# uguryagmur/RealTimeObjectDetection

Hardware: AMD Instinct MI355X
Metric: frames/sec YOLOv3 608x608 bs=8 (Darknet.forward + write_results; 2 batches in flight, write_results_async on a second stream) (higher is better)
Workload: dtype f16x2-split (3 MFMA products, f32 accumulate); 1 GPU; YOLOv3 cfg 608x608 batch=8 per GPU, split-f16 MFMA conv + fused head + GPU NMS (BASELINE configs[2]); precision=f16s3, tiles=autotune (this run), parallelism=frame-shard x1, in_flight_batches=2, detections_last_step=1699, candidates_last_step=1914, f16_range_overflow=False

## Files before the change

### realtimeobjectdetection_amd/csrc/conv_f16s3_common.h

```cpp
#pragma once
#include "rtod_internal.h"
#include <type_traits>

namespace rtod {

typedef float f32x4 __attribute__((ext_vector_type(4)));
typedef _Float16 f16x8 __attribute__((ext_vector_type(8)));
typedef unsigned int u32x4 __attribute__((ext_vector_type(4)));

constexpr int HBK = 32;
constexpr unsigned OOB = 0x80000000u;


template <int N> __device__ __forceinline__ void vmcnt() {
    static_assert(0 <= N && N <= 63, "vmcnt range");
    asm volatile("s_waitcnt vmcnt(%0)" :: "n"(N) : "memory");
}

template <int OFF = 0> __device__ __forceinline__ u32x4 buffer_load_b128(const __amdgpu_buffer_rsrc_t rsrc, unsigned voffset, unsigned soffset) {
    u32x4 v;
    asm volatile("buffer_load_dwordx4 %0, %1, %2, %3 offen offset:%4" : "=v"(v) : "v"(voffset), "s"(rsrc), "s"(soffset), "n"(OFF) : "memory");
    return v;
}

// ... 169 lines not shown
        if (kg == 1) return;
#pragma unroll
        for (int i = 0; i < TM; ++i)
#pragma unroll
            for (int j = 0; j < TN; ++j) {
                const f32x4 o = T[base + (i * TN + j) * 64];
#pragma unroll
                for (int e = 0; e < 4; ++e) acc[i][j][e] += o[e];
            }
    }
    float amax = 0.f;
    _Float16* const oh = reinterpret_cast<_Float16*>(a.out) + a.out_coff;
    const _Float16* const rh = reinterpret_cast<const _Float16*>(a.res) + a.res_coff;
#pragma unroll
    for (int P = 0; P < NP; ++P) {
        const int c0 = cbase + 32 * P + 8 * lh;
        const bool cok = c0 < a.Cout;
        const int cc = cok ? c0 : 0;
        f16x8 rq_h[RES ? TM : 1], rq_l[RES ? TM : 1];
        if constexpr (RES) {
#pragma unroll
            for (int i = 0; i < TM; ++i) {
                const int m = mrow[i];
                const bool ok = m >= 0 && cok;
                const _Float16* q = rh + (int64_t)(ok ? m : 0) * 2 * a.res_ldc + cc;
                rq_h[i] = ok ? *reinterpret_cast<const f16x8*>(q) : f16x8{0, 0, 0, 0, 0, 0, 0, 0};
                rq_l[i] = ok ? *reinterpret_cast<const f16x8*>(q + a.res_ldc) : f16x8{0, 0, 0, 0, 0, 0, 0, 0};
            }
        }
        f32x4 iv0 = *reinterpret_cast<const f32x4*>(a.inv_scale + cc), iv1 = *reinterpret_cast<const f32x4*>(a.inv_scale + cc + 4);
        f32x4 bs0 = *reinterpret_cast<const f32x4*>(a.bias + cc), bs1 = *reinterpret_cast<const f32x4*>(a.bias + cc + 4);
#pragma unroll
        for (int i = 0; i < TM; ++i) {
            const int m = mrow[i];
            f16x8 ph, pl;
#pragma unroll
            for (int e = 0; e < 8; ++e) {
                const float s = e < 4 ? acc[i][2 * P][e] : acc[i][2 * P + 1][e - 4];
                float v = s * ((e < 4 ? iv0[e] : iv1[e - 4]) * SPLIT_SCALE) + (e < 4 ? bs0[e] : bs1[e - 4]) * SPLIT_SCALE;
                if (a.leaky) v = v > 0.f ? v : v * 0.1f;
                if constexpr (RES) v += (float)rq_h[i][e] + (float)rq_l[i][e];
                _Float16 h, l;
                split_f16(v, h, l, amax);
                ph[e] = h; pl[e] = l;
            }
            if (m >= 0 && cok) {
                _Float16* q = oh + (int64_t)m * 2 * a.out_ldc + c0;
                store_act16(q, ph, false);
                store_act16(q + a.out_ldc, pl, false);
            }
        }
    }
    split_overflow_report(a.ovf, amax);
}

constexpr int epi_row_group(int bm, int wm, int rg_max) {
    int best = wm;
    for (int r = wm; r <= bm && r <= rg_max; r += wm) if (bm % r == 0) best = r;
    return best;
}


template <int BM, int BN, int WM, int WN, int NT, int EPI, int SMEM_BYTES, int KG = 1, bool PRE = false, bool F16 = false, bool RAW = false>
__device__ __forceinline__ void conv_f16s3_epilogue(const ConvArgs& a, f32x4 (&acc)[WM / 16][WN / 16], unsigned char* smem,
                                                    int bm, int bn, int tid, int wm, int wn, int lr, int lh, int M, int kg = 0,
                                                    const float* pre_bias = nullptr, const float* pre_inv = nullptr) {
    constexpr int MT = 16, TM = WM / MT, TN = WN / MT;
    constexpr bool PW = EPI == EPI_SPLIT_PW || EPI == EPI_SPLIT_RES_PW;
    constexpr bool RES = EPI == EPI_SPLIT_RES || EPI == EPI_SPLIT_RES_PW;
    static_assert(!(F16 && PW), "plain-f16 plans host no pointwise conv");
    static_assert(!RAW || (EPI == EPI_SPLIT && !F16), "raw-sum instances: no shortcut, decode, hosted pointwise conv or plain-f16 store");
    constexpr int TS = PW ? BN + 4 : BN;
    constexpr int T2S = PW_MAX_COUT + 4;
    constexpr int RG_MAX = SMEM_BYTES / ((TS + (PW ? T2S : 0)) * 4);
    constexpr int RG = epi_row_group(BM, WM, RG_MAX);
    static_assert(RG >= WM && BM % RG == 0, "epilogue row group");
    static_assert(RG * (TS + (PW ? T2S : 0)) * 4 <= SMEM_BYTES, "epilogue tile exceeds the kernel's LDS");
    float* T = reinterpret_cast<float*>(smem);
    const int hw = a.Ho * a.Wo;
#ifdef RTOD_DIAG
    const bool st_plain = (a.dbg & 8) != 0;
#else
    constexpr bool st_plain = false;
#endif
    float amax = 0.f;
    constexpr int PWK = PW_MAX_K / 32;
    f16x8 b2h[PW ? PWK : 1], b2l[PW ? PWK : 1];
    float bias2 = 0.f, inv2 = 0.f;
    int pw_n2t = 1, pw_j = 0;
    if constexpr (PW) {
        pw_n2t = a.pw_cout / 16;
        pw_j = (tid >> 6) % pw_n2t;
        const int n2 = pw_j * 16 + (tid & 15);
        const _Float16* w2h = a.pw_wh + (int64_t)n2 * 32 + ((tid & 63) >> 4) * 8;
        const _Float16* w2l = a.pw_wl + (int64_t)n2 * 32 + ((tid & 63) >> 4) * 8;
#pragma unroll
        for (int ks = 0; ks < PWK; ++ks) {
            const bool ok = ks * 32 < a.pw_k;
            b2h[ks] = ok ? *reinterpret_cast<const f16x8*>(w2h + (int64_t)ks * a.pw_npad * 32) : f16x8{0, 0, 0, 0, 0, 0, 0, 0};
            b2l[ks] = ok ? *reinterpret_cast<const f16x8*>(w2l + (int64_t)ks * a.pw_npad * 32) : f16x8{0, 0, 0, 0, 0, 0, 0, 0};
        }
        bias2 = a.pw_bias[n2] * SPLIT_SCALE; inv2 = a.pw_inv_scale[n2] * SPLIT_SCALE;
    }
    const float escale = (EPI == EPI_DECODE || RAW) ? 1.0f : SPLIT_SCALE;
    constexpr int GPR_ = BN / 8;
    constexpr int NG = (RG * GPR_ + NT - 1) / NT;
// ... 174 lines not shown
```

### realtimeobjectdetection_amd/csrc/conv_pwd_f16s3.hip

```cpp
#include "conv_bandd_common.h"

namespace rtod {

template <int BM, int NW, int NST, int MINW, int EPI>
__global__ __launch_bounds__(NW * 64, MINW)
void conv_pwd_f16s3_kernel(const ConvArgs a, const int grid_m, const int grid_n) {
    constexpr bool F16 = epi_f16(EPI);
    constexpr int LB = F16 ? 2 : 4, LP = F16 ? 1 : 2;
    constexpr int BN = NW * 32, NT = NW * 64, TM = BM / 16, TN = 2;
    constexpr int SLAB = BM * 256;
    constexpr int NP = BM / 8;
    constexpr int NPP = (NP + NW - 1) / NW;
    static_assert(BM % 16 == 0 && NPP >= 1 && NPP <= 8, "slab pieces per wave");
    static_assert(NST >= 2 && NST <= 4, "ring depth");
    constexpr int RG = BM * BN * 4 <= 32768 ? BM : (BM / 2) * BN * 4 <= 32768 ? BM / 2 : BM / 4;
    constexpr int WAIT_B = 2 * LB + LP * NPP;
    constexpr int WAIT_SLAB = 2 * LB + (NST - 2) * (LP * NPP + 2 * LB);
    constexpr int WAIT_SLAB_PRO = 2 * LB + (NST - 2) * LP * NPP;

    extern __shared__ __attribute__((aligned(16))) unsigned char smem[];
    const int nwg = grid_m * grid_n;
    int bid = blockIdx.x;
    if (!a.xcd_by_n) bid = xcd_remap(bid, nwg);
    const int bm = bid / grid_n, bn = bid - bm * grid_n;
    const int tid = (int)threadIdx.x;
    const int wave = __builtin_amdgcn_readfirstlane(tid >> 6), lane = tid & 63;
    const int lr = lane & 15, lh = lane >> 4;
    const int M = a.B * a.Hi * a.Wi;
    const int m0 = bm * BM;
    const unsigned PS = (unsigned)a.in_ldc * 4u;
    const unsigned lo_plane = (unsigned)a.in_ldc * 2u;

    const __amdgpu_buffer_rsrc_t rs_a = buffer_rsrc(a.in, a.in_bytes);
    const __amdgpu_buffer_rsrc_t rs_wh = buffer_rsrc(a.w_hi, a.w_bytes);
    const __amdgpu_buffer_rsrc_t rs_wl = buffer_rsrc(a.w_lo, a.w_bytes);
    const unsigned lds0 = (unsigned)(size_t)smem;
    const int NS = a.Cin / 64;

    unsigned dma_vo[NPP];
#pragma unroll
    for (int k = 0; k < NPP; ++k) {
        const int p = wave + k * NW;
        const int r = lane >> 3;
        const int m = m0 + p * 8 + r;
        dma_vo[k] = (p < NP && m < M) ? (unsigned)m * PS + (unsigned)(a.in_coff + (((lane & 7) ^ r) << 3)) * 2u : OOB;
    }
    auto dma_slab = [&](int js) __attribute__((always_inline)) {
        const bool live = js < NS;
        const unsigned soff = (unsigned)js * 128u;
        const unsigned base = lds0 + (unsigned)((js % NST) * SLAB);
#pragma unroll
        for (int k = 0; k < NPP; ++k) {
            const int p = wave + k * NW;
            const unsigned dst = p < NP ? base + (unsigned)((p >> 1) * 4096 + (p & 1) * 1024) : lds0 + (unsigned)(NST * SLAB);
            if constexpr (F16) lds_dma(rs_a, live ? dma_vo[k] : OOB, soff, dst);
// ... 34 lines not shown
        if constexpr (!F16) l = *reinterpret_cast<lds_f16x8*>((unsigned)(o + 4096 * i + 2048));
    };

#pragma unroll
    for (int s = 0; s < NST - 1; ++s) dma_slab(s);
    load_b(0, Bq[0]);
    load_b(1, Bq[1]);

    __builtin_amdgcn_s_setprio(2);
    auto slab_body = [&](int j, auto par_c) __attribute__((always_inline)) {
        constexpr int par = decltype(par_c)::value;
        asm volatile("" : "+v"(xq0), "+v"(xq1));
        if (j < NST - 1) vmcnt<WAIT_SLAB_PRO>(); else vmcnt<WAIT_SLAB>();
        __builtin_amdgcn_sched_barrier(0);
        __builtin_amdgcn_s_barrier();
        dma_slab(j + NST - 1);
        const int slotoff = (int)lds0 + (j % NST) * SLAB;
        read_unit(0, 0, slotoff, Ah[0], Al[0]);
        read_unit(1 / TM, 1 % TM, slotoff, Ah[1], Al[1]);
        __builtin_amdgcn_sched_barrier(0);
#pragma unroll
        for (int u = 0; u < 2 * TM; ++u) {
            const int q = u / TM, i = u % TM;
            if (i == 0) {
                if (q == 0) load_b(2 * j + 2, Bq[(2 * par + 2) % 4]); else load_b(2 * j + 3, Bq[(2 * par + 3) % 4]);
                vmcnt<WAIT_B>();
                if (q == 0) tie_bset<F16>(Bq[2 * par]); else tie_bset<F16>(Bq[2 * par + 1]);
                __builtin_amdgcn_sched_barrier(0);
            }
            if (u + 2 < 2 * TM) read_unit((u + 2) / TM, (u + 2) % TM, slotoff, Ah[(u + 2) % 3], Al[(u + 2) % 3]);
            const f16x8 ah = Ah[u % 3], al = Al[u % 3];
#pragma unroll
            for (int jn = 0; jn < TN; ++jn) {
                const f16x8 bh = __builtin_bit_cast(f16x8, Bq[2 * par + q][jn][0]);
                if constexpr (F16) { acc[i][jn] = __builtin_amdgcn_mfma_f32_16x16x32_f16(ah, bh, acc[i][jn], 0, 0, 0); continue; }
                const f16x8 bl = __builtin_bit_cast(f16x8, Bq[2 * par + q][jn][1]);
                acc[i][jn] = __builtin_amdgcn_mfma_f32_16x16x32_f16(al, bh, acc[i][jn], 0, 0, 0);
                acc[i][jn] = __builtin_amdgcn_mfma_f32_16x16x32_f16(ah, bl, acc[i][jn], 0, 0, 0);
                acc[i][jn] = __builtin_amdgcn_mfma_f32_16x16x32_f16(ah, bh, acc[i][jn], 0, 0, 0);
            }
            __builtin_amdgcn_sched_barrier(0);
        }
    };
#pragma unroll 1
    for (int j = 0; j < NS; j += 2) {
        slab_body(j, std::integral_constant<int, 0>{});
        if (j + 1 < NS) slab_body(j + 1, std::integral_constant<int, 1>{});
    }
    vmcnt<0>();
    tie_bset<F16>(Bq[0]); tie_bset<F16>(Bq[1]); tie_bset<F16>(Bq[2]); tie_bset<F16>(Bq[3]);
    __builtin_amdgcn_sched_barrier(0);
    __builtin_amdgcn_s_setprio(0);

    bandd_epilogue<BM, BN, BM, 32, NT, RG, epi_kind(EPI) == EPI_SPLIT_RES, 1, F16, epi_raw(EPI)>(a, acc, smem, bm, bn, tid, 0, wn, lr, lh, M, 0);
}

template <int BM, int NW, int NST, int MINW>
static int launch_pwd(const ConvArgs& a, hipStream_t s) {
    constexpr int BN = NW * 32, NT = NW * 64;
    constexpr int RG = BM * BN * 4 <= 32768 ? BM : (BM / 2) * BN * 4 <= 32768 ? BM / 2 : BM / 4;
    const int M = a.B * a.Ho * a.Wo;
    const int gm = (M + BM - 1) / BM, gn = (a.Cout + BN - 1) / BN;
    ConvArgs ax = a;
    ax.xcd_by_n = (gn % 8 == 0 && (int64_t)a.Cout * a.K > (int64_t)M * a.Cin) ? 1 : 0;
    constexpr int ring_bytes = NST * BM * 256 + ((BM / 8) % NW ? 4096 : 0), epi_bytes = RG * BN * 4;
    constexpr int lds = ring_bytes > epi_bytes ? ring_bytes : epi_bytes;
    static_assert(lds <= 160 * 1024, "LDS");
    const int fe = a.f16 ? 1 : 0;
    auto k_res = fe ? conv_pwd_f16s3_kernel<BM, NW, NST, MINW, EPI_SPLIT_RES | EPI_F16> : conv_pwd_f16s3_kernel<BM, NW, NST, MINW, EPI_SPLIT_RES>;
    auto k_plain = fe ? conv_pwd_f16s3_kernel<BM, NW, NST, MINW, EPI_SPLIT | EPI_F16> : conv_pwd_f16s3_kernel<BM, NW, NST, MINW, EPI_SPLIT>;
    auto k_raw = conv_pwd_f16s3_kernel<BM, NW, NST, MINW, EPI_SPLIT | EPI_RAW>;
    if constexpr (lds > 64 * 1024) {
        static std::atomic<unsigned long long> attr_done[3] = {{0}, {0}, {0}};
        if (a.raw_out) { if (int rc = lds_opt_in(attr_done[2], lds, "conv_pwd_f16s3", k_raw)) return rc; }
        else if (int rc = lds_opt_in(attr_done[fe], lds, "conv_pwd_f16s3", k_res, k_plain)) return rc;
    }
    if (a.raw_out) {
        hipLaunchKernelGGL(k_raw, dim3(gm * gn), dim3(NT), lds, s, ax, gm, gn);
        return hip_fail(hipGetLastError(), "conv_pwd_f16s3 launch");
    }
    if (a.res) hipLaunchKernelGGL(k_res, dim3(gm * gn), dim3(NT), lds, s, ax, gm, gn);
    else hipLaunchKernelGGL(k_plain, dim3(gm * gn), dim3(NT), lds, s, ax, gm, gn);
    return hip_fail(hipGetLastError(), "conv_pwd_f16s3 launch");
}

#define RTOD_PWD_TILES(X) \
    X(0, 64, 4, 3, 3) X(1, 32, 4, 3, 3) X(2, 128, 4, 3, 1) X(3, 64, 8, 3, 1) X(4, 64, 4, 2, 3) X(5, 32, 4, 4, 3) X(6, 96, 4, 2, 3) X(7, 96, 4, 3, 2) X(8, 48, 4, 3, 3) X(9, 48, 4, 4, 3) X(10, 64, 2, 2, 4)

#define RTOD_X_INFO(idx, bm, nw, nst, minw) {bm, nw * 32, "conv_pwd_f16s3<" #bm "x" #nw "w,r" #nst ">"},
static const ConvVariantInfo kPwdModes[PWD_MODES] = { RTOD_PWD_TILES(RTOD_X_INFO) };
#undef RTOD_X_INFO
const ConvVariantInfo& conv_pwd_mode_info(int idx) { return kPwdModes[idx < 0 || idx >= PWD_MODES ? 0 : idx]; }

bool conv_pwd_supported(int ksize, int stride, int pad, int cin) { return ksize == 1 && stride == 1 && pad == 0 && cin >= 64 && cin % 64 == 0; }

int conv_pwd_kernel_name(int idx, int epi, char* buf, size_t len) {
#define RTOD_X_NAME(i, bm, nw, nst, minw) \
    if (idx == i) return snprintf(buf, len, "void rtod::conv_pwd_f16s3_kernel<" #bm ", " #nw ", " #nst ", " #minw ", %d>(rtod::ConvArgs, int, int)", epi);
    RTOD_PWD_TILES(RTOD_X_NAME)
#undef RTOD_X_NAME
    return -1;
}

int launch_conv_pwd_f16s3(const ConvArgs& a, int idx, hipStream_t s) {
    if (int rc = check_split_conv_args(a, "launch_conv_pwd", true)) return rc;
    if (!conv_pwd_supported(a.kh, a.stride, a.pad, a.Cin) || a.kw != 1 || a.Ho != a.Hi || a.Wo != a.Wi || a.dec.enabled || a.pw_wh) {
        set_error("launch_conv_pwd: unsupported shape (k=%d s=%d pad=%d Cin=%d)", a.kh, a.stride, a.pad, a.Cin); return RTOD_E_ARG;
    }
    if (a.in_ldc % 8 || a.in_coff % 8 || a.K != a.Kpad || a.K != a.Cin || a.Npad % 128) { set_error("launch_conv_pwd: bad view / K"); return RTOD_E_ARG; }
    if (a.raw_out && (a.f16 || a.res)) { set_error("launch_conv_pwd: a raw-sum launch carries no shortcut and no plain-f16 store"); return RTOD_E_ARG; }
    if (a.raw_out && a.raw_ld != a.Npad) { set_error("launch_conv_pwd: raw-sum rows are Npad floats in this family (raw_ld %d, Npad %d)", a.raw_ld, a.Npad); return RTOD_E_ARG; }
    switch (idx) {
#define RTOD_X_CASE(i, bm, nw, nst, minw) case i: return launch_pwd<bm, nw, nst, minw>(a, s);
        RTOD_PWD_TILES(RTOD_X_CASE)
#undef RTOD_X_CASE
    }
    set_error("launch_conv_pwd: mode %d unsupported", idx);
    return RTOD_E_ARG;
}

}
```

### realtimeobjectdetection_amd/csrc/plan_tiles.cpp

```cpp
#include "plan.h"

#include <algorithm>
#include <mutex>

namespace rtod {

int Plan::choose_variant(const Layer& L, int batch) const {
    if (opt_force_f32_variant >= 0 && opt_force_f32_variant < CV_COUNT) return opt_force_f32_variant;
    if (L.cout <= 32) return CV_128x32;
    if (L.cout <= 64) return CV_128x64;
    const int64_t M = (int64_t)batch * L.hout * L.wout;
    const int64_t big = ((M + 127) / 128) * ((L.cout + 127) / 128);
    return big >= 512 ? CV_128x128 : CV_64x64;
}

int Plan::f32_slice_mode(const Launch& l, int batch, int variant) const {
    const PackedConv& pc = convs[l.conv_slot];
    if (pc.split || pc.stem || pc.slice_chunks <= 0) return 0;
    const Layer& L = layers[l.layer];
    const ConvVariantInfo& vi = conv_variant_info(variant);
    const int64_t M = (int64_t)batch * L.hout * L.wout;
    const int64_t tiles = ((M + vi.bm - 1) / vi.bm) * ((L.cout + vi.bn - 1) / vi.bn);
    const int64_t S = (pc.Kpad / 32 + pc.slice_chunks - 1) / pc.slice_chunks;
    return (opt_k_slice_workgroups && d_scratch && tiles < 512 && S * M * pc.Npad <= scratch_floats) ? 2 : 1;
}

bool Plan::tile_legal(const Launch& l, int v) const {
    const TileRef t = family_of(v);
    if (!t || l.kind != LK_CONV || l.conv_slot < 0 || !convs[l.conv_slot].split) return false;
    const PackedConv& pc = convs[l.conv_slot];
    const Layer& L = layers[l.layer];
    if (precision == 2 && !t.f16()) return false;
    if (raw_launch(l) && !t.raw()) return false;
    if (pc.narrow || t.is(TF_C16)) return pc.narrow && t.is(TF_C16);
    if (pc.ks_chunks > 0 || t.is(TF_KS)) return pc.ks_chunks > 0 && t.is(TF_KS);
    if (pc.band) return t.is(TF_BAND) && conv_band_mode_valid(t.mode, L.cin, L.hin, L.win);
    const bool hosts_pw = form(&l - &launches[0]).guest >= 0, plain = l.out_layer != -2 && !hosts_pw, same_map = L.hout == L.hin && L.wout == L.win;
    switch (t.fam->id) {
        case TF_GENERIC: return !(hosts_pw && t.fam->info(t.mode).bn < L.cout);
        case TF_BAND: return t.bandd_wide() && opt_band_kernel && plain && same_map && pc.Npad % 128 == 0 && pc.K == pc.Kpad &&
                             conv_bandd_wide_supported(L.size, L.stride, L.pad, pc.cin_p, L.win);
        case TF_RING: return !hosts_pw && L.act <= 1;
        case TF_PWD: return opt_pwd_kernel && plain && same_map && conv_pwd_supported(L.size, L.stride, L.pad, pc.cin_p);
        case TF_PATCH: return plain && L.act <= 1 && L.hout == L.hin && conv_patch_supported(L.size, L.stride, L.pad, L.cin, L.cout) &&
                              conv_patch_mode_valid(t.mode, L.cin, L.cout);
    }
    return false;
}

int Plan::default_tile(const Launch& l, int batch) const {
    const PackedConv& pc = convs[l.conv_slot];
    const Layer& L = layers[l.layer];
    const int64_t M = (int64_t)batch * L.hout * L.wout;
    if (pc.narrow) return tile_id(TF_C16, conv_c16_default_mode(L.cout, M));
    if (pc.ks_chunks > 0) return tile_id(TF_KS, ((M + 63) / 64) * ((L.cout + 63) / 64) < 512 ? 1 : 0);
    if (pc.band) {
        if (precision != 2 && !raw_launch(l)) return tile_id(TF_BAND, conv_band_default_mode(L.cin, L.hin, L.win));
        const TileFamily& B = tile_family(TF_BAND);
        for (int m = 0; m < B.modes; ++m) if (tile_legal(l, B.base + m)) return B.base + m;
        return B.base + B.f16_from;
    }
    const int64_t gn = (L.cout + 127) / 128;
    const int g = L.cout <= 64 ? HV_128x64 : ((M + 127) / 128) * gn >= 512 ? HV_128x128 : ((M + 63) / 64) * gn >= 512 ? HV_64x128 : HV_64x64;
    return tile_legal(l, g) ? g : HV_128x128_8W;
}

int Plan::variant_for(const Launch& l, int batch) const {
    int want = opt_force_f16s3_variant;
    if (want < 0) {
        auto it = tuned.find(batch);
        const size_t idx = &l - &launches[0];
        if (it != tuned.end() && idx < it->second.size()) want = it->second[idx];
    }
    int v = want >= 0 && tile_legal(l, want) ? want : default_tile(l, batch);
    if (family_of(v).ks_sched_b() && !(opt_k_slice_workgroups && ks_sched_b_fits(l, batch))) --v;
    return v;
}

std::vector<int> Plan::tile_candidates(const Launch& l, int batch) const {
    static const int kOrder[TF_COUNT] = {TF_GENERIC, TF_PATCH, TF_BAND, TF_PWD, TF_RING, TF_C16, TF_KS};
    const int cout = layers[l.layer].cout;
    const bool ks_b = opt_k_slice_workgroups && ks_sched_b_fits(l, batch);
    std::vector<int> cand;
    for (int f : kOrder) {
        if ((f == TF_RING && !opt_ring_kernel) || (f == TF_PATCH && !opt_patch_kernel)) continue;
        const TileFamily& F = tile_family(f);
        for (int m = 0; m < F.modes; ++m) {
            const int bn = F.info(m).bn;
            const bool too_wide = f == TF_GENERIC || f == TF_RING ? bn > 64 && bn > 2 * ((cout + 63) / 64 * 64)
                                : f == TF_PATCH ? bn > 64 && bn > cout
                                : f == TF_PWD ? bn > 128 && bn > (cout + 127) / 128 * 128 : false;
            if (too_wide || (family_of(F.base + m).ks_sched_b() && !ks_b) || !tile_legal(l, F.base + m)) continue;
            cand.push_back(F.base + m);
        }
    }
    return cand;
}

int Plan::launch_split_variant(ConvArgs& a, const PackedConv& pc, int v, hipStream_t s) const {
    const TileRef t = family_of(v);
    if (!t) { set_error("variant %d is no split-f16 tile", v); return RTOD_E_STATE; }
    if (precision == 2 && !t.f16()) { set_error("variant %d has no plain-f16 instance", v); return RTOD_E_STATE; }
    if (a.raw_out && !t.raw()) { set_error("variant %d has no raw-sum instance", v); return RTOD_E_STATE; }
    if (pc.narrow != t.is(TF_C16)) {
        set_error(pc.narrow ? "variant %d requested for a narrow (Cin = 16) layer" : "narrow variant %d requested for a layer without tap-major weights", v);
        return RTOD_E_STATE;
    }
    if ((pc.ks_chunks > 0) != t.is(TF_KS)) {
        set_error(pc.ks_chunks > 0 ? "variant %d requested for a K-sliced layer" : "K-sliced variant %d requested for a layer that is not sliced", v);
        return RTOD_E_STATE;
    }
    if (pc.band != t.is(TF_BAND) && !(t.bandd_wide() && !pc.band)) {
        set_error(pc.band ? "variant %d requested for a band layer" : "band variant %d requested for a layer without band weights", v);
        return RTOD_E_STATE;
    }
    if (t.is(TF_KS)) {
        a.slice_chunks = pc.ks_chunks;
        a.partial = nullptr; a.partial_floats = 0;
        if (t.ks_sched_b()) { a.partial = d_scratch; a.partial_floats = scratch_floats; }
    }
    return t.fam->launch(a, t.mode, s);
}

static std::mutex g_tune_mutex;
static std::map<std::vector<int>, int> g_tune_memo;

int Plan::tune_launch(size_t li, ConvArgs& a, int batch, hipStream_t s) {
    const Launch& l = launches[li];
    const Layer& L = layers[l.layer];
    const bool pw = a.pw_wh != nullptr;
    const std::vector<int> key = {L.cin, L.cout, L.size, L.stride, L.hout, L.wout, l.in2_layer >= 0, l.out_layer == -2, pw ? a.pw_cout : 0,
                                  convs[l.conv_slot].band ? 1 : 0, opt_ring_kernel ? 1 : 0, opt_patch_kernel ? 1 : 0, opt_pwd_kernel ? 1 : 0, L.act,
                                  precision, L.hin, L.win, L.pad, convs[l.conv_slot].ks_chunks, opt_k_slice_workgroups ? 1 : 0,
                                  a.raw_out ? 1 : 0};
    auto it = tune_cache.find(key);
    if (it != tune_cache.end()) { tuning[li] = it->second; return RTOD_OK; }
    std::vector<int> gkey = key; gkey.push_back(device); gkey.push_back(batch);
    {
        std::lock_guard<std::mutex> lock(g_tune_mutex);
        auto git = g_tune_memo.find(gkey);
        if (git != g_tune_memo.end()) { tuning[li] = git->second; tune_cache[key] = git->second; return RTOD_OK; }
    }
    hipEvent_t e0, e1;
    RTOD_HIP(hipEventCreate(&e0)); RTOD_HIP(hipEventCreate(&e1));
    const std::vector<int> cand = tile_candidates(l, batch);
    int best_v = variant_for(l, batch);
    int rc = RTOD_OK;
    auto time_variant = [&](int v, int reps, int per, float& out_ms) -> int {
        out_ms = 1e30f;
        for (int rep = 0; rep < reps; ++rep) {
            (void)hipEventRecord(e0, s);
            for (int r = 0; r < per; ++r) { const int q = launch_split_variant(a, convs[l.conv_slot], v, s); if (q) return q; }
            (void)hipEventRecord(e1, s);
            if (hipEventSynchronize(e1) != hipSuccess) return hip_fail(hipGetLastError(), "autotune sync");
            float ms = 0.f; (void)hipEventElapsedTime(&ms, e0, e1);
            out_ms = std::min(out_ms, ms / per);
        }
        return RTOD_OK;
    };
    std::vector<std::pair<float, int>> ranked;
    for (int v : cand) {
        rc = launch_split_variant(a, convs[l.conv_slot], v, s);
        if (rc) break;
        float ms; rc = time_variant(v, 3, 2, ms);
        if (rc) break;
        ranked.push_back({ms, v});
    }
    if (!rc && !ranked.empty()) {
        std::sort(ranked.begin(), ranked.end());
        const size_t top = std::min<size_t>(3, ranked.size());
        std::vector<float> fin(top, 1e30f);
        for (int round = 0; round < 5 && !rc; ++round)
            for (size_t t = 0; t < top && !rc; ++t) {
                float ms; rc = time_variant(ranked[t].second, 2, 4, ms);
                fin[t] = std::min(fin[t], ms);
            }
        if (!rc) best_v = ranked[std::min_element(fin.begin(), fin.end()) - fin.begin()].second;
    }
    (void)hipEventDestroy(e0); (void)hipEventDestroy(e1);
    if (rc) return rc;
    tuning[li] = best_v;
    tune_cache[key] = best_v;
    { std::lock_guard<std::mutex> lock(g_tune_mutex); g_tune_memo[gkey] = best_v; }
    return RTOD_OK;
}

int Plan::set_tiles(int batch, const int* variants, int count) {
// ... 27 lines not shown
```

### realtimeobjectdetection_amd/csrc/rtod_internal.h

```cpp
#pragma once
#include <hip/hip_runtime.h>
#if defined(RTOD_STAMPS) && !defined(RTOD_DIAG)
#define RTOD_DIAG 1
#endif
#include <algorithm>
#include <atomic>
#include <cstdint>
#include <cstdio>
#include <string>
#include <vector>

#include "../../include/rtod.h"

namespace rtod {

void set_error(const char* fmt, ...);
int hip_fail(hipError_t e, const char* what);

#define RTOD_HIP(expr)                                              \
    do {                                                            \
        hipError_t _e = (expr);                                     \
        if (_e != hipSuccess) return ::rtod::hip_fail(_e, #expr);   \
    } while (0)

// ... 98 lines not shown
}
__device__ __forceinline__ __amdgpu_buffer_rsrc_t buffer_rsrc(const void* p, unsigned bytes) {
    return __builtin_amdgcn_make_buffer_rsrc(const_cast<void*>(p), 0, bytes, 0x00020000);
}
__device__ __forceinline__ int xcd_remap(int id, int n) {
    const int q = n >> 3, r = n & 7, xcd = id & 7;
    return (xcd < r ? xcd * (q + 1) : r * (q + 1) + (xcd - r) * q) + (id >> 3);
}
#endif

constexpr int EPI_F16 = 8;
constexpr int EPI_RAW = 16;

enum ConvVariant { CV_128x128 = 0, CV_128x64 = 1, CV_64x64 = 2, CV_128x32 = 3, CV_COUNT };
struct ConvVariantInfo { int bm, bn; const char* name; };
const ConvVariantInfo& conv_variant_info(int v);
int conv_f32_kernel_name(int variant, char* buf, size_t len);
int launch_conv(const ConvArgs& a, int variant, hipStream_t s);
int conv_f32_slices(const ConvArgs& a);
enum ConvF16Variant { HV_128x128 = 0, HV_128x64 = 1, HV_64x64 = 2, HV_64x128 = 3, HV_256x128 = 4, HV_128x256 = 5, HV_128x128_8W = 6, HV_128x64_8W = 7, HV_256x128_16W = 8,
                      HV_192x128_8W = 9, HV_96x128_8W = 10, HV_192x128_12W = 11, HV_COUNT };
const ConvVariantInfo& conv_f16s3_variant_info(int v);
int conv_f16s3_kernel_name(int variant, int epi, char* buf, size_t len);
int launch_conv_f16s3(const ConvArgs& a, int variant, hipStream_t s);
bool conv_band_supported(int ksize, int stride, int pad, int cin, int w_in);
constexpr int BANDD_MODES = 9;
constexpr int BAND_LDS_MODES = 11;
constexpr int BAND_MODES = BAND_LDS_MODES + BANDD_MODES;
constexpr int BAND_K2_MODE0 = 7;
const ConvVariantInfo& conv_bandd_mode_info(int idx);
int conv_bandd_mode_kg(int idx);
constexpr int BANDD_WIDE_MODE = BAND_LDS_MODES + 7;
bool conv_bandd_wide_supported(int ksize, int stride, int pad, int cin, int w_in);
int conv_bandd_kernel_name(int idx, int epi, char* buf, size_t len);
int launch_conv_bandd_f16s3(const ConvArgs& a, int idx, hipStream_t s);
int conv_band_layer_kg(int cin, int h, int w);
bool conv_band_mode_valid(int mode, int cin, int h, int w);
int conv_band_default_mode(int cin, int h, int w);
const ConvVariantInfo& conv_band_mode_info(int mode);
int conv_band_kernel_name(int mode, int epi, char* buf, size_t len);
int launch_conv_band_f16s3(const ConvArgs& a, int mode, hipStream_t s);
constexpr int BAND_VARIANT_BASE = 50;
constexpr int RING_MODES = 8;
constexpr int RING_VARIANT_BASE = 70;
const ConvVariantInfo& conv_ring_mode_info(int mode);
int conv_ring_kernel_name(int mode, int epi, char* buf, size_t len);
int launch_conv_ring_f16s3(const ConvArgs& a, int mode, hipStream_t s);
constexpr int PWD_MODES = 11;
constexpr int PWD_VARIANT_BASE = 90;
bool conv_pwd_supported(int ksize, int stride, int pad, int cin);
const ConvVariantInfo& conv_pwd_mode_info(int mode);
int conv_pwd_kernel_name(int mode, int epi, char* buf, size_t len);
int launch_conv_pwd_f16s3(const ConvArgs& a, int mode, hipStream_t s);
constexpr int STEM2_VARIANT = 130;
bool conv_stem2_supported(int k0, int s0, int p0, int cin0, int cout0, int k1, int s1, int p1, int cout1, int pw_cout);
int conv_stem2_kernel_name(int pw, char* buf, size_t len);
int launch_conv_stem2_f16s3(const float* x, int B, int H, int W, const _Float16* w0h, const _Float16* w0l, const float* inv0, const float* bias0,
                            int leaky0, const ConvArgs& c1, hipStream_t s);
constexpr int PATCH_MODES = 5;
constexpr int PATCH_WRES_MODE = 4;
bool conv_patch_mode_valid(int mode, int cin, int cout);
constexpr int PATCH_VARIANT_BASE = 110;
bool conv_patch_supported(int ksize, int stride, int pad, int cin, int cout);
const ConvVariantInfo& conv_patch_mode_info(int mode);
int conv_patch_kernel_name(int mode, int epi, char* buf, size_t len);
int launch_conv_patch_f16s3(const ConvArgs& a, int mode, hipStream_t s);

constexpr int C16_MODES = 4;
constexpr int C16_VARIANT_BASE = 140;
constexpr bool conv_c16_supported(int cin) { return cin == 16; }
const ConvVariantInfo& conv_c16_mode_info(int mode);
int conv_c16_default_mode(int cout, int64_t m);
int conv_c16_kernel_name(int mode, int epi, char* buf, size_t len);
int launch_conv_c16_f16s3(const ConvArgs& a, int mode, hipStream_t s);

constexpr int KS_TILES = 3;
constexpr int KS_MODES = 2 * KS_TILES;
constexpr int KS_VARIANT_BASE = 150;
constexpr int64_t KS_SCRATCH_FLOATS = 8ll << 20;
const ConvVariantInfo& conv_ks_mode_info(int mode);
int conv_ks_slices(const ConvArgs& a);
int conv_ks_kernel_name(int mode, int epi, char* buf, size_t len);
int launch_conv_ks_f16s3(const ConvArgs& a, int mode, hipStream_t s);

enum TileFamilyId { TF_GENERIC = 0, TF_BAND, TF_RING, TF_PWD, TF_PATCH, TF_C16, TF_KS, TF_COUNT };
struct TileFamily {
    int id, base, modes;
    int f16_from;
    int raw_from;
    const ConvVariantInfo& (*info)(int mode);
    int (*kernel_name)(int mode, int epi, char* buf, size_t len);
    int (*launch)(const ConvArgs& a, int mode, hipStream_t s);
};
struct TileRef {
    const TileFamily* fam; int mode;
    explicit operator bool() const { return fam != nullptr; }
    bool is(int family) const { return fam && fam->id == family; }
    bool f16() const { return fam && mode >= fam->f16_from; }
    bool raw() const { return fam && mode >= fam->raw_from; }
    bool ks_sched_b() const { return is(TF_KS) && (mode & 1); }
    bool bandd_wide() const { return is(TF_BAND) && mode == BANDD_WIDE_MODE; }
};
TileRef family_of(int v);
const TileFamily& tile_family(int family);
inline int tile_id(int family, int mode) { return tile_family(family).base + mode; }

int launch_conv_stem(const float* x_nchw, const float* w, const float* bias, const View& out, int B, int H, int W,
                     int Ho, int Wo, int stride, int Cout, int leaky, hipStream_t s);
int launch_conv_stem_split(const float* x_nchw, const _Float16* wh, const _Float16* wl, const float* inv_scale, const float* bias,
                           const View& out, int B, int H, int W, int Ho, int Wo, int stride, int Cout, int leaky, int32_t* ovf, hipStream_t s);
bool conv_stem16_supported(int ksize, int stride, int pad, int cin, int cout, int act);
int launch_conv_stem16_f16s3(const float* x_nchw, const _Float16* wh, const _Float16* wl, const float* inv_scale, const float* bias,
                             const View& out, int B, int H, int W, int act, int pool, int32_t* ovf, hipStream_t s);
int launch_conv_stem16_raw(const float* x_nchw, const _Float16* wh, const _Float16* wl, const float* inv_scale, const View& raw, int B, int H, int W, hipStream_t s);
int launch_prep_image(const unsigned char* img, int h, int w, int bgr, int inp_dim, float* out, hipStream_t s);
int launch_prep_frames(const unsigned char* frames, int batch, int h, int w, int bgr, int out_h, int out_w, float* out, hipStream_t s);
int launch_pack_input(const float* x_nchw, int B, int C, int H, int W, float* out_nhwc, int Cp, hipStream_t s);
int launch_upsample2x(const View& in, const View& out, int B, hipStream_t s);
int launch_add(const View& a, const View& b, const View& out, int B, hipStream_t s, int32_t* ovf = nullptr);
int launch_maxpool(const View& in, const View& out, int B, int size, int stride, int pad, hipStream_t s);
int launch_upsample_nearest2x(const View& in, const View& out, int B, hipStream_t s);
int launch_bn_batch(const View& x, const View& y, const View* res, int B, double* stats, int sstride, const float* bn, int gstride, int act,
                    double* partial, int64_t partial_doubles, hipStream_t s);
size_t bn_partial_doubles(int max_channels);
int launch_bn_batch_split(const View& raw, const View& y, const View* res, int B, double* stats, int sstride, const float* bn, int gstride, int act,
                          double* partial, int64_t partial_doubles, int32_t* ovf, hipStream_t s, int pool = 0);
struct BnUpdateEntry { float* running_mean; float* running_var; int64_t stats_off; double unbias; int sstride; int channels; };
constexpr int BN_UPDATE_MAX = 32;
struct BnUpdateTable { BnUpdateEntry e[BN_UPDATE_MAX]; };
int launch_bn_update_running(const BnUpdateEntry* entries, int n, const double* stats, double momentum, hipStream_t s);
int launch_copy(const View& in, const View& out, int B, hipStream_t s);
int launch_view_to_nchw(const View& in, int B, float* out_nchw, hipStream_t s);
int launch_finish_decode(float* out, int B, const DecodeArgs& d, int hw_exp, hipStream_t s);
int launch_decode(const float* raw, int64_t sb, int64_t sc, int64_t sy, int64_t sx, int B,
                  const DecodeArgs& d, float* out, hipStream_t s);
int launch_confidence_mask(const float* pred, int64_t rows, int attrs, float conf, float* out, hipStream_t s);
int launch_bbox_iou(const float* box1, const float* boxes, int k, int row_stride, float* iou, hipStream_t s);

// ... 57 lines not shown
```

### realtimeobjectdetection_amd/csrc/split_tiles.cpp

```cpp
#include "rtod_internal.h"

namespace rtod {

static const TileFamily kFamilies[TF_COUNT] = {
    {TF_GENERIC, 0, HV_COUNT, 0, 0, conv_f16s3_variant_info, conv_f16s3_kernel_name, launch_conv_f16s3},
    {TF_BAND, BAND_VARIANT_BASE, BAND_MODES, BAND_LDS_MODES, BAND_LDS_MODES, conv_band_mode_info, conv_band_kernel_name, launch_conv_band_f16s3},
    {TF_RING, RING_VARIANT_BASE, RING_MODES, RING_MODES, RING_MODES, conv_ring_mode_info, conv_ring_kernel_name, launch_conv_ring_f16s3},
    {TF_PWD, PWD_VARIANT_BASE, PWD_MODES, 0, 0, conv_pwd_mode_info, conv_pwd_kernel_name, launch_conv_pwd_f16s3},
    {TF_PATCH, PATCH_VARIANT_BASE, PATCH_MODES, PATCH_MODES, PATCH_MODES, conv_patch_mode_info, conv_patch_kernel_name, launch_conv_patch_f16s3},
    {TF_C16, C16_VARIANT_BASE, C16_MODES, 0, 0, conv_c16_mode_info, conv_c16_kernel_name, launch_conv_c16_f16s3},
    {TF_KS, KS_VARIANT_BASE, KS_MODES, 0, KS_MODES, conv_ks_mode_info, conv_ks_kernel_name, launch_conv_ks_f16s3},
};
static_assert(HV_COUNT <= BAND_VARIANT_BASE, "generic tile ids end where the band family's begin");
static_assert(BAND_VARIANT_BASE + BAND_MODES <= RING_VARIANT_BASE, "band tile ids end where the ring family's begin");
static_assert(RING_VARIANT_BASE + RING_MODES <= PWD_VARIANT_BASE, "ring tile ids end where the pwd family's begin");
static_assert(PWD_VARIANT_BASE + PWD_MODES <= PATCH_VARIANT_BASE, "pwd tile ids end where the patch family's begin");
static_assert(PATCH_VARIANT_BASE + PATCH_MODES <= STEM2_VARIANT && STEM2_VARIANT < C16_VARIANT_BASE, "the fused stem's reported id lies between the patch and narrow families");
static_assert(C16_VARIANT_BASE + C16_MODES <= KS_VARIANT_BASE, "narrow tile ids end where the K-sliced family's begin");

TileRef family_of(int v) {
    for (const TileFamily& f : kFamilies)
        if (v >= f.base && v < f.base + f.modes) return {&f, v - f.base};
    return {nullptr, 0};
}

const TileFamily& tile_family(int family) { return kFamilies[family]; }

}
```

Baseline: 2550 frames/s.

## Add pointwise slab conv family with fused YOLOv3 decode epilogue for head layers

Adds a new tile family (TF_PWDH) that runs the 1x1 detection-head convolutions through the slab-ring pointwise kernel and applies the YOLOv3 box decode (sigmoid/exp/anchor/grid offset) in its epilogue, writing straight into the detection buffer. Previously head layers could not use the pwd kernel because it rejected decode launches, so they fell back to other families. The autotuner now sees these extra candidates for head layers. This adds template instances and a per-row index walk in the epilogue, and the tune cache key gains a field.

```diff
diff --git a/realtimeobjectdetection_amd/csrc/conv_f16s3_common.h b/realtimeobjectdetection_amd/csrc/conv_f16s3_common.h
--- a/realtimeobjectdetection_amd/csrc/conv_f16s3_common.h
+++ b/realtimeobjectdetection_amd/csrc/conv_f16s3_common.h
@@ -245,6 +245,23 @@
         }
     }
     split_overflow_report(a.ovf, amax);
+}
+
+struct DecodeCol { int c; bool is_wh, is_raw; float anc; };
+__device__ __forceinline__ DecodeCol epi_decode_col(const ConvArgs& a, int n) {
+    const int an = n / a.dec.attrs, c = n - an * a.dec.attrs;
+    const bool is_wh = (c == 2 || c == 3) && !a.dec.train;
+    const bool is_raw = (c == 2 || c == 3) && a.dec.train;
+    const float anc = (c == 2 ? a.dec.aw[an] : a.dec.ah[an]);
+    return {c, is_wh, is_raw, anc};
+}
+__device__ __forceinline__ float epi_decode1(const DecodeArgs& d, const DecodeCol& k, float v, int gx, int gy) {
+    const float ex = __expf(k.is_wh ? v : -v);
+    const float wh = (ex * k.anc) * d.stride;
+    const float sg = __builtin_amdgcn_rcpf(1.0f + ex);
+    const float xy = (sg + (float)(k.c == 0 ? gx : gy)) * d.stride;
+    const float o = k.is_wh ? wh : (k.c < 2 && !d.train) ? xy : sg;
+    return k.is_raw ? v : o;
 }
 
 constexpr int epi_row_group(int bm, int wm, int rg_max) {
diff --git a/realtimeobjectdetection_amd/csrc/conv_pwd_f16s3.hip b/realtimeobjectdetection_amd/csrc/conv_pwd_f16s3.hip
--- a/realtimeobjectdetection_amd/csrc/conv_pwd_f16s3.hip
+++ b/realtimeobjectdetection_amd/csrc/conv_pwd_f16s3.hip
@@ -1,6 +1,59 @@
 #include "conv_bandd_common.h"
 
 namespace rtod {
+
+template <int BM, int BN, int NT, int RG>
+__device__ __forceinline__ void pwd_decode_epilogue(const ConvArgs& a, f32x4 (&acc)[BM / 16][2], unsigned char* smem, int bm, int bn, int tid,
+                                                    int wn, int lr, int lh, int M) {
+    constexpr int WM = BM, WN = 32, TM = WM / 16, TN = WN / 16, MT = 16, TS = BN, KG = 1;
+    constexpr bool RAW = false;
+    constexpr int wm = 0, kg = 0;
+    static_assert(BM % RG == 0 && RG % 16 == 0, "epilogue pass");
+    static_assert(BN % 64 == 0 && NT % BN == 0 && RG % (NT / BN) == 0, "decode mapping: a wave reads 64 columns of one row, rows advance by NT / BN");
+    constexpr int RSTEP = NT / BN, NR = RG / RSTEP;
+    float* T = reinterpret_cast<float*>(smem);
+    const float escale = 1.0f;
+    float bias_j[TN], inv_j[TN];
+#pragma unroll
+    for (int j = 0; j < TN; ++j) epi_col_params(a, bn * BN + wn * WN + j * MT + lr, bias_j[j], inv_j[j]);
+    const int nl = tid % BN, r0 = __builtin_amdgcn_readfirstlane(tid / BN);
+    const int n = bn * BN + nl;
+    const bool live = n < a.Cout;
+    const DecodeCol col = epi_decode_col(a, live ? n : 0);
+    const int hw = a.Ho * a.Wo;
+    const float* Tp = T + r0 * TS + nl;
+    const int64_t img_fix = a.dec.img_stride - (int64_t)hw * a.Cout;
+    __syncthreads();
+#pragma unroll
+    for (int rg = 0; rg < BM; rg += RG) {
+#define EPI_WAVE_IN_PASS true
+#define EPI_TILE_IN_PASS(i) (wm * WM + (i) * MT >= rg && wm * WM + (i) * MT < rg + RG)
+#define EPI_TILE_ROW(i) (wm * WM + (i) * MT - rg)
+#include "conv_f16s3_epi_transpose.inc"
+#undef EPI_WAVE_IN_PASS
+#undef EPI_TILE_IN_PASS
+#undef EPI_TILE_ROW
+        __syncthreads();
+        float v[NR];
+#pragma unroll
+        for (int k = 0; k < NR; ++k) v[k] = Tp[k * RSTEP * TS];
+        int m = bm * BM + rg + r0;
+        const int b = m / hw;
+        int cell = m - b * hw;
+        int gy = cell / a.dec.GW, gx = cell - gy * a.dec.GW;
+        float* row = a.out + (int64_t)b * a.dec.img_stride + a.dec.head_off + (int64_t)cell * a.Cout;
+        if (live) {
+            for (int k = 0; k < NR; ++k) {
+                if (m >= M) break;
+                row[n] = epi_decode1(a.dec, col, v[k], gx, gy);
+                m += RSTEP; cell += RSTEP; gx += RSTEP; row += RSTEP * a.Cout;
+                while (gx >= a.dec.GW) { gx -= a.dec.GW; ++gy; }
+                while (cell >= hw) { cell -= hw; gy -= a.dec.GH; row += img_fix; }
+            }
+        }
+        if (rg + RG < BM) __syncthreads();
+    }
+}
 
 template <int BM, int NW, int NST, int MINW, int EPI>
 __global__ __launch_bounds__(NW * 64, MINW)
@@ -141,19 +194,25 @@
     __builtin_amdgcn_sched_barrier(0);
     __builtin_amdgcn_s_setprio(0);
 
-    bandd_epilogue<BM, BN, BM, 32, NT, RG, epi_kind(EPI) == EPI_SPLIT_RES, 1, F16, epi_raw(EPI)>(a, acc, smem, bm, bn, tid, 0, wn, lr, lh, M, 0);
+    if constexpr (epi_kind(EPI) == EPI_DECODE) pwd_decode_epilogue<BM, BN, NT, RG>(a, acc, smem, bm, bn, tid, wn, lr, lh, M);
+    else bandd_epilogue<BM, BN, BM, 32, NT, RG, epi_kind(EPI) == EPI_SPLIT_RES, 1, F16, epi_raw(EPI)>(a, acc, smem, bm, bn, tid, 0, wn, lr, lh, M, 0);
+}
+
+template <int BM, int NW, int NST> constexpr int pwd_lds_bytes() {
+    constexpr int BN = NW * 32;
+    constexpr int RG = BM * BN * 4 <= 32768 ? BM : (BM / 2) * BN * 4 <= 32768 ? BM / 2 : BM / 4;
+    constexpr int ring_bytes = NST * BM * 256 + ((BM / 8) % NW ? 4096 : 0), epi_bytes = RG * BN * 4;
+    return ring_bytes > epi_bytes ? ring_bytes : epi_bytes;
 }
 
 template <int BM, int NW, int NST, int MINW>
 static int launch_pwd(const ConvArgs& a, hipStream_t s) {
     constexpr int BN = NW * 32, NT = NW * 64;
-    constexpr int RG = BM * BN * 4 <= 32768 ? BM : (BM / 2) * BN * 4 <= 32768 ? BM / 2 : BM / 4;
     const int M = a.B * a.Ho * a.Wo;
     const int gm = (M + BM - 1) / BM, gn = (a.Cout + BN - 1) / BN;
     ConvArgs ax = a;
     ax.xcd_by_n = (gn % 8 == 0 && (int64_t)a.Cout * a.K > (int64_t)M * a.Cin) ? 1 : 0;
-    constexpr int ring_bytes = NST * BM * 256 + ((BM / 8) % NW ? 4096 : 0), epi_bytes = RG * BN * 4;
-    constexpr int lds = ring_bytes > epi_bytes ? ring_bytes : epi_bytes;
+    constexpr int lds = pwd_lds_bytes<BM, NW, NST>();
     static_assert(lds <= 160 * 1024, "LDS");
     const int fe = a.f16 ? 1 : 0;
     auto k_res = fe ? conv_pwd_f16s3_kernel<BM, NW, NST, MINW, EPI_SPLIT_RES | EPI_F16> : conv_pwd_f16s3_kernel<BM, NW, NST, MINW, EPI_SPLIT_RES>;
@@ -191,6 +250,51 @@
     return -1;
 }
 
+template <int BM, int NW, int NST, int MINW>
+static int launch_pwdh(const ConvArgs& a, hipStream_t s) {
+    constexpr int BN = NW * 32, NT = NW * 64;
+    const int M = a.B * a.Ho * a.Wo;
+    const int gm = (M + BM - 1) / BM, gn = (a.Cout + BN - 1) / BN;
+    constexpr int lds = pwd_lds_bytes<BM, NW, NST>();
+    static_assert(lds <= 64 * 1024, "LDS without the opt-in");
+    hipLaunchKernelGGL((conv_pwd_f16s3_kernel<BM, NW, NST, MINW, EPI_DECODE>), dim3(gm * gn), dim3(NT), lds, s, a, gm, gn);
+    return hip_fail(hipGetLastError(), "conv_pwd_f16s3 head launch");
+}
+
+#define RTOD_PWDH_TILES(X) X(0, 64, 8, 3, 1) X(1, 96, 4, 2, 3) X(2, 48, 4, 3, 3) X(3, 32, 4, 3, 3)
+
+#define RTOD_X_INFO(idx, bm, nw, nst, minw) {bm, nw * 32, "conv_pwd_f16s3<" #bm "x" #nw "w,r" #nst ",decode>"},
+static const ConvVariantInfo kPwdhModes[PWDH_MODES] = { RTOD_PWDH_TILES(RTOD_X_INFO) };
+#undef RTOD_X_INFO
+const ConvVariantInfo& conv_pwdh_mode_info(int idx) { return kPwdhModes[idx < 0 || idx >= PWDH_MODES ? 0 : idx]; }
+
+int conv_pwdh_kernel_name(int idx, int epi, char* buf, size_t len) {
+#define RTOD_X_NAME(i, bm, nw, nst, minw) \
+    if (idx == i) return snprintf(buf, len, "void rtod::conv_pwd_f16s3_kernel<" #bm ", " #nw ", " #nst ", " #minw ", %d>(rtod::ConvArgs, int, int)", epi);
+    RTOD_PWDH_TILES(RTOD_X_NAME)
+#undef RTOD_X_NAME
+    return -1;
+}
+
+int launch_conv_pwdh_f16s3(const ConvArgs& a, int idx, hipStream_t s) {
+    if (int rc = check_split_conv_args(a, "launch_conv_pwdh", false)) return rc;
+    if (!conv_pwd_supported(a.kh, a.stride, a.pad, a.Cin) || a.kw != 1 || a.Ho != a.Hi || a.Wo != a.Wi) {
+        set_error("launch_conv_pwdh: unsupported shape (k=%d s=%d pad=%d Cin=%d)", a.kh, a.stride, a.pad, a.Cin); return RTOD_E_ARG;
+    }
+    if (!a.dec.enabled || a.dec.v5 || a.dec.attrs <= 0 || a.dec.GW <= 0 || a.dec.GH * a.dec.GW != a.Ho * a.Wo || a.Cout > a.dec.attrs * 4) {
+        set_error("launch_conv_pwdh: a fused YOLOv3-style decode of this map only"); return RTOD_E_ARG;
+    }
+    if (a.f16 || a.raw_out || a.res || a.pw_wh) { set_error("launch_conv_pwdh: f16s3 only, no shortcut, no raw sums, no hosted pointwise conv"); return RTOD_E_ARG; }
+    if (a.in_ldc % 8 || a.in_coff % 8 || a.K != a.Kpad || a.K != a.Cin || a.Npad % 128 || a.Cout > a.Npad) { set_error("launch_conv_pwdh: bad view / K"); return RTOD_E_ARG; }
+    switch (idx) {
+#define RTOD_X_CASE(i, bm, nw, nst, minw) case i: return launch_pwdh<bm, nw, nst, minw>(a, s);
+        RTOD_PWDH_TILES(RTOD_X_CASE)
+#undef RTOD_X_CASE
+    }
+    set_error("launch_conv_pwdh: mode %d unsupported", idx);
+    return RTOD_E_ARG;
+}
+
 int launch_conv_pwd_f16s3(const ConvArgs& a, int idx, hipStream_t s) {
     if (int rc = check_split_conv_args(a, "launch_conv_pwd", true)) return rc;
     if (!conv_pwd_supported(a.kh, a.stride, a.pad, a.Cin) || a.kw != 1 || a.Ho != a.Hi || a.Wo != a.Wi || a.dec.enabled || a.pw_wh) {
diff --git a/realtimeobjectdetection_amd/csrc/plan_tiles.cpp b/realtimeobjectdetection_amd/csrc/plan_tiles.cpp
--- a/realtimeobjectdetection_amd/csrc/plan_tiles.cpp
+++ b/realtimeobjectdetection_amd/csrc/plan_tiles.cpp
@@ -44,6 +44,7 @@
         case TF_PWD: return opt_pwd_kernel && plain && same_map && conv_pwd_supported(L.size, L.stride, L.pad, pc.cin_p);
         case TF_PATCH: return plain && L.act <= 1 && L.hout == L.hin && conv_patch_supported(L.size, L.stride, L.pad, L.cin, L.cout) &&
                               conv_patch_mode_valid(t.mode, L.cin, L.cout);
+        case TF_PWDH: return opt_pwd_kernel && l.out_layer == -2 && !l.dec.v5 && !hosts_pw && same_map && conv_pwd_supported(L.size, L.stride, L.pad, pc.cin_p);
     }
     return false;
 }
@@ -78,7 +79,7 @@
 }
 
 std::vector<int> Plan::tile_candidates(const Launch& l, int batch) const {
-    static const int kOrder[TF_COUNT] = {TF_GENERIC, TF_PATCH, TF_BAND, TF_PWD, TF_RING, TF_C16, TF_KS};
+    static const int kOrder[TF_COUNT] = {TF_GENERIC, TF_PATCH, TF_BAND, TF_PWD, TF_PWDH, TF_RING, TF_C16, TF_KS};
     const int cout = layers[l.layer].cout;
     const bool ks_b = opt_k_slice_workgroups && ks_sched_b_fits(l, batch);
     std::vector<int> cand;
@@ -89,7 +90,7 @@
             const int bn = F.info(m).bn;
             const bool too_wide = f == TF_GENERIC || f == TF_RING ? bn > 64 && bn > 2 * ((cout + 63) / 64 * 64)
                                 : f == TF_PATCH ? bn > 64 && bn > cout
-                                : f == TF_PWD ? bn > 128 && bn > (cout + 127) / 128 * 128 : false;
+                                : f == TF_PWD || f == TF_PWDH ? bn > 128 && bn > (cout + 127) / 128 * 128 : false;
             if (too_wide || (family_of(F.base + m).ks_sched_b() && !ks_b) || !tile_legal(l, F.base + m)) continue;
             cand.push_back(F.base + m);
         }
@@ -114,6 +115,10 @@
         set_error(pc.band ? "variant %d requested for a band layer" : "band variant %d requested for a layer without band weights", v);
         return RTOD_E_STATE;
     }
+    if (t.is(TF_PWDH) && (!a.dec.enabled || a.dec.v5 || a.pw_wh)) {
+        set_error("head slab variant %d requested for a launch without a fused YOLOv3-style decode", v);
+        return RTOD_E_STATE;
+    }
     if (t.is(TF_KS)) {
         a.slice_chunks = pc.ks_chunks;
         a.partial = nullptr; a.partial_floats = 0;
@@ -132,7 +137,8 @@
     const std::vector<int> key = {L.cin, L.cout, L.size, L.stride, L.hout, L.wout, l.in2_layer >= 0, l.out_layer == -2, pw ? a.pw_cout : 0,
                                   convs[l.conv_slot].band ? 1 : 0, opt_ring_kernel ? 1 : 0, opt_patch_kernel ? 1 : 0, opt_pwd_kernel ? 1 : 0, L.act,
                                   precision, L.hin, L.win, L.pad, convs[l.conv_slot].ks_chunks, opt_k_slice_workgroups ? 1 : 0,
-                                  a.raw_out ? 1 : 0};
+                                  a.raw_out ? 1 : 0,
+                                  l.out_layer == -2 && l.dec.v5 ? 1 : 0};
     auto it = tune_cache.find(key);
     if (it != tune_cache.end()) { tuning[li] = it->second; return RTOD_OK; }
     std::vector<int> gkey = key; gkey.push_back(device); gkey.push_back(batch);
diff --git a/realtimeobjectdetection_amd/csrc/rtod_internal.h b/realtimeobjectdetection_amd/csrc/rtod_internal.h
--- a/realtimeobjectdetection_amd/csrc/rtod_internal.h
+++ b/realtimeobjectdetection_amd/csrc/rtod_internal.h
@@ -174,6 +174,11 @@
 const ConvVariantInfo& conv_pwd_mode_info(int mode);
 int conv_pwd_kernel_name(int mode, int epi, char* buf, size_t len);
 int launch_conv_pwd_f16s3(const ConvArgs& a, int mode, hipStream_t s);
+constexpr int PWDH_MODES = 4;
+constexpr int PWDH_VARIANT_BASE = 170;
+const ConvVariantInfo& conv_pwdh_mode_info(int mode);
+int conv_pwdh_kernel_name(int mode, int epi, char* buf, size_t len);
+int launch_conv_pwdh_f16s3(const ConvArgs& a, int mode, hipStream_t s);
 constexpr int STEM2_VARIANT = 130;
 bool conv_stem2_supported(int k0, int s0, int p0, int cin0, int cout0, int k1, int s1, int p1, int cout1, int pw_cout);
 int conv_stem2_kernel_name(int pw, char* buf, size_t len);
@@ -205,7 +210,7 @@
 int conv_ks_kernel_name(int mode, int epi, char* buf, size_t len);
 int launch_conv_ks_f16s3(const ConvArgs& a, int mode, hipStream_t s);
 
-enum TileFamilyId { TF_GENERIC = 0, TF_BAND, TF_RING, TF_PWD, TF_PATCH, TF_C16, TF_KS, TF_COUNT };
+enum TileFamilyId { TF_GENERIC = 0, TF_BAND, TF_RING, TF_PWD, TF_PATCH, TF_C16, TF_KS, TF_PWDH, TF_COUNT };
 struct TileFamily {
     int id, base, modes;
     int f16_from;
diff --git a/realtimeobjectdetection_amd/csrc/split_tiles.cpp b/realtimeobjectdetection_amd/csrc/split_tiles.cpp
--- a/realtimeobjectdetection_amd/csrc/split_tiles.cpp
+++ b/realtimeobjectdetection_amd/csrc/split_tiles.cpp
@@ -10,6 +10,7 @@
     {TF_PATCH, PATCH_VARIANT_BASE, PATCH_MODES, PATCH_MODES, PATCH_MODES, conv_patch_mode_info, conv_patch_kernel_name, launch_conv_patch_f16s3},
     {TF_C16, C16_VARIANT_BASE, C16_MODES, 0, 0, conv_c16_mode_info, conv_c16_kernel_name, launch_conv_c16_f16s3},
     {TF_KS, KS_VARIANT_BASE, KS_MODES, 0, KS_MODES, conv_ks_mode_info, conv_ks_kernel_name, launch_conv_ks_f16s3},
+    {TF_PWDH, PWDH_VARIANT_BASE, PWDH_MODES, PWDH_MODES, PWDH_MODES, conv_pwdh_mode_info, conv_pwdh_kernel_name, launch_conv_pwdh_f16s3},
 };
 static_assert(HV_COUNT <= BAND_VARIANT_BASE, "generic tile ids end where the band family's begin");
 static_assert(BAND_VARIANT_BASE + BAND_MODES <= RING_VARIANT_BASE, "band tile ids end where the ring family's begin");
@@ -17,6 +18,7 @@
 static_assert(PWD_VARIANT_BASE + PWD_MODES <= PATCH_VARIANT_BASE, "pwd tile ids end where the patch family's begin");
 static_assert(PATCH_VARIANT_BASE + PATCH_MODES <= STEM2_VARIANT && STEM2_VARIANT < C16_VARIANT_BASE, "the fused stem's reported id lies between the patch and narrow families");
 static_assert(C16_VARIANT_BASE + C16_MODES <= KS_VARIANT_BASE, "narrow tile ids end where the K-sliced family's begin");
+static_assert(KS_VARIANT_BASE + KS_MODES <= PWDH_VARIANT_BASE, "K-sliced tile ids end where the head slab family's begin");
 
 TileRef family_of(int v) {
     for (const TileFamily& f : kFamilies)
```

Measured after the change: 2564 frames/s (median of 4 runs). No clear change (+0.5%).
